# rust-cv/cv

Hardware: NVIDIA H100
Metric: vSLAM frames/s (AKAZE+match+RANSAC, 1080p ~5k kp) at 1/2/4/8 H100 (higher is better)
Workload: dtype f32+f64

## Files before the change

### cv_b200/csrc/arrsac_dev.cuh

```cuda
#pragma once

#define ARS_SORT_CAP 4096u
#define ARS_BOOK_NT 1024
#define ARS_BOOK_SMEM (14u * ARS_SORT_CAP)
#define ARS_QCAP (1u << 20)

struct ArrsacCtl {
    uint32_t n, init_n, Mv, npass;
    uint32_t Hn, cur, blk_lo, blk_hi;
    uint32_t acc_hi, n_new, worst, done;
    uint32_t found, iters, nraw, q_count;
    uint32_t q_count2, stat_lazy;
    uint32_t stat_units0, stat_units2;
    uint32_t stat_repairs, stat_pad;
    uint64_t rng_pos, gen_pos;
    cvb_rng gen;
    cvb_pose winner;
    uint32_t n_inliers, overflow;
    uint32_t stat_chunks, stat_pass;
    uint32_t stat_walk_us, stat_commit_us;
    uint32_t stat_perm_us, stat_turns;
    uint32_t q_blk, stat_qblk;
};

struct ArrsacParams {
    uint32_t K, MM, kind;
    uint32_t H0, ib, bs, max_cand, G;
    uint32_t W0;
    uint32_t NW;
    uint32_t NMAX;
    uint32_t rows;
    uint32_t prefix, cmin;
    float lr_thr, eps0, delta0;
    double thr;
    int row0;
};

__device__ __forceinline__ unsigned long long ars_globaltimer() { unsigned long long t; asm volatile("mov.u64 %0, %%globaltimer;" : "=l"(t)); return t; }
__device__ __forceinline__ uint64_t ars_rotl64(uint64_t x, int k) { return (x << k) | (x >> (64 - k)); }
__device__ uint32_t ars_rng_next_u32(cvb_rng *r) {
    if (r->kind == 0) {
        uint64_t *s = r->s;
        const uint64_t result = ars_rotl64(s[0] + s[3], 23) + s[0];
        const uint64_t t = s[1] << 17;
        s[2] ^= s[0]; s[3] ^= s[1]; s[1] ^= s[2]; s[0] ^= s[3]; s[2] ^= t; s[3] = ars_rotl64(s[3], 45);
        return (uint32_t)(result >> 32);
    }
    unsigned __int128 state = (unsigned __int128)r->s[0] | ((unsigned __int128)r->s[1] << 64);
    const unsigned __int128 incr = (unsigned __int128)r->s[2] | ((unsigned __int128)r->s[3] << 64);
    const unsigned __int128 MUL = ((unsigned __int128)0x2360ED051FC65DA4ull << 64) | 0x4385DF649FCCF645ull;
    state = state * MUL + incr;
    r->s[0] = (uint64_t)state; r->s[1] = (uint64_t)(state >> 64);
    const uint32_t rot = (uint32_t)(state >> 122);
    const uint64_t xsl = (uint64_t)(state >> 64) ^ (uint64_t)state;
    return (uint32_t)((xsl >> rot) | (xsl << ((64 - rot) & 63)));
}

__device__ uint32_t ars_raw_at(ArrsacCtl *ctl, const uint32_t *raw, uint64_t pos) {
    if (pos < ctl->nraw) return raw[pos];
    uint32_t v = 0;
    while (ctl->gen_pos <= pos) { v = ars_rng_next_u32(&ctl->gen); ctl->gen_pos++; }
    return v;
}

#define ARS_WIN 4096u
// ... 150 lines not shown
__global__ void __launch_bounds__(128, MINB) k_ars_estimate8(const ArrsacCtl *ctl, int phase, uint32_t H_init, const double *__restrict__ a,
                                                       const double *__restrict__ b, const uint32_t *__restrict__ samples,
                                                       cvb_pose *poses, uint8_t *nposes) {
    if (ctl->done) return;
    __shared__ double sh[(128 / EIGHT_LANES) * EIGHT_SH];
    const uint32_t H = phase == 0 ? H_init : ctl->n_new;
    const uint32_t g = threadIdx.x / EIGHT_LANES, lane = threadIdx.x % EIGHT_LANES;
    const uint32_t h = blockIdx.x * (128 / EIGHT_LANES) + g;
    if (h >= H) return;
    const unsigned mask = ((1u << EIGHT_LANES) - 1u) << ((threadIdx.x & 31) / EIGHT_LANES * EIGHT_LANES);
    cvb_pose out[4];
    const int n = eight_point_lanes<EIGHT_LANES>(a, b, samples + (size_t)h * 8, out, sh + g * EIGHT_SH, lane, mask);
    if (lane == 0) {
        for (int k = 0; k < n; k++) poses[(size_t)h * 4 + k] = out[k];
        nposes[h] = (uint8_t)n;
    }
}

__device__ __noinline__ bool ars_exact_c2c(const cvb_pose *Pz, const double *pa, const double *pb, double thr) {
    return residual_c2c(*Pz, pa, pb) < thr;
}

template <int RES>
__device__ __forceinline__ bool ars_inlier(const cvb_pose &Pz, const double *__restrict__ a, const double *__restrict__ b, uint32_t i,
                                           double thr) {
    if (RES == 1) return residual_w2c(Pz, a + 3 * (size_t)i, b + 4 * (size_t)i) < thr;
    const double *pa = a + 3 * (size_t)i, *pb = b + 3 * (size_t)i;
    int f = c2c_inlier_filter(Pz.r, Pz.t, pa, pb, thr);
    if (f < 0) f = ars_exact_c2c(&Pz, pa, pb, thr) ? 1 : 0;
    return f != 0;
}

template <int RES>
__device__ __forceinline__ bool ars_inlier_queued(const cvb_pose &Pz, const double *__restrict__ a, const double *__restrict__ b, uint32_t i,
                                                  double thr, uint32_t *qc, uint2 *q, uint32_t src) {
    if (RES == 1) return ars_inlier<RES>(Pz, a, b, i, thr);
    const double *pa = a + 3 * (size_t)i, *pb = b + 3 * (size_t)i;
    const int f = c2c_inlier_filter(Pz.r, Pz.t, pa, pb, thr);
    if (f >= 0) return f != 0;
    const uint32_t slot = atomicAdd(qc, 1u);
    if (slot < ARS_QCAP) { q[slot] = make_uint2(src, i); return false; }
    return ars_exact_c2c(&Pz, pa, pb, thr);
}

__device__ __forceinline__ bool ars_ready(uint32_t word0, uint32_t init_n, uint32_t sample, const ArrsacParams &P) {
    if (sample < P.prefix) return true;
    const uint32_t c = min(32u, init_n);
    return (uint32_t)__popc(c < 32 ? (word0 & ((1u << c) - 1)) : word0) >= P.cmin;
}

template <int RES>
__global__ void __launch_bounds__(256, 2) k_ars_score(ArrsacCtl *ctl, uint2 *__restrict__ queue, ArrsacParams P, int phase, const double *__restrict__ a,
                                                   const double *__restrict__ b, const cvb_pose *__restrict__ poses0,
                                                   const uint8_t *__restrict__ nposes0, uint32_t *__restrict__ masks0,
                                                   const cvb_pose *__restrict__ tposes, uint32_t *__restrict__ tmasks,
                                                   const cvb_pose *__restrict__ newposes, const uint8_t *__restrict__ nposes_new,
                                                   uint32_t *__restrict__ newmask) {
    if (ctl->done) return;
    const unsigned full = 0xffffffffu;
    const uint32_t lane = threadIdx.x & 31;
    const uint32_t warp = (blockIdx.x * blockDim.x + threadIdx.x) >> 5, nwarps = (gridDim.x * blockDim.x) >> 5;
    if (phase == 0 || phase == 2) {
        const uint32_t init_n = ctl->init_n, W = (init_n + 31) >> 5;
        const uint32_t nmod = P.H0 * P.MM, npre = min(P.prefix, P.H0) * P.MM, W1 = W > 0 ? W - 1 : 0;
        const uint32_t units = phase == 0 ? nmod + npre * W1 : (nmod - npre) * W1;
        uint32_t *qc = phase == 0 ? &ctl->q_count : &ctl->q_count2;
        uint2 *q = phase == 0 ? queue : queue + ARS_QCAP;
        for (uint32_t u = warp; u < units; u += nwarps) {
            uint32_t m, w;
            if (phase == 0) { if (u < nmod) { m = u; w = 0; } else { m = (u - nmod) / W1; w = 1 + (u - nmod) % W1; } }
            else { m = npre + u / W1; w = 1 + u % W1; }
            if ((m % P.MM) >= nposes0[m / P.MM]) continue;
            if (phase == 2 && !ars_ready(masks0[(size_t)m * P.W0], init_n, m / P.MM, P)) continue;
            const uint32_t i = w * 32 + lane;
            bool bit = false;
            if (i < init_n) bit = ars_inlier_queued<RES>(poses0[m], a, b, i, P.thr, qc, q, m);
            const unsigned bits = __ballot_sync(full, bit);
            if (lane == 0) { masks0[(size_t)m * P.W0 + w] = bits; atomicAdd(phase == 0 ? &ctl->stat_units0 : &ctl->stat_units2, 1u); }
        }
        return;
    }
    const uint32_t lo = ctl->blk_lo, hi = ctl->blk_hi, Hn = ctl->Hn, cur = ctl->cur;
    const uint32_t wlo = lo >> 5, nwb = hi > lo ? ((hi - 1) >> 5) - wlo + 1 : 0;
    const uint32_t kept_units = Hn * nwb;
    const uint32_t nnew = ctl->n_new * P.MM, nwn = (hi + 31) >> 5;
    const uint32_t units = kept_units + nnew * nwn;
    const cvb_pose *tp = tposes + (size_t)cur * P.rows;
    uint32_t *tm = tmasks + (size_t)cur * P.rows * P.NW;
    for (uint32_t u = warp; u < units; u += nwarps) {
        if (u < kept_units) {
            const uint32_t r = u / nwb, w = wlo + u % nwb;
            const uint32_t i = w * 32 + lane;
            const bool act = i >= lo && i < hi;
            bool bit = false;
            if (act) bit = ars_inlier_queued<RES>(tp[r], a, b, i, P.thr, &ctl->q_blk, queue, r);
            const unsigned bits = __ballot_sync(full, bit), range = __ballot_sync(full, act);
            if (lane == 0) { uint32_t *p = tm + (size_t)r * P.NW + w; *p = (*p & ~range) | bits; }
        } else {
            const uint32_t v = u - kept_units;
            const uint32_t j = v / nwn, w = v % nwn;
            if ((j % P.MM) >= nposes_new[j / P.MM]) continue;
            const uint32_t i = w * 32 + lane;
            bool bit = false;
            if (i < hi) bit = ars_inlier_queued<RES>(newposes[j], a, b, i, P.thr, &ctl->q_blk, queue, P.rows + j);
            const unsigned bits = __ballot_sync(full, bit);
            if (lane == 0) newmask[(size_t)j * P.NW + w] = bits;
        }
    }
}

__global__ void __launch_bounds__(256) k_ars_resolve(const ArrsacCtl *ctl, const uint2 *__restrict__ queue, int stage, ArrsacParams P,
                                                     const double *__restrict__ a, const double *__restrict__ b,
                                                     const cvb_pose *__restrict__ poses0, uint32_t *__restrict__ masks0) {
    if (ctl->done) return;
    const uint32_t cnt = min(stage == 0 ? ctl->q_count : ctl->q_count2, ARS_QCAP);
    queue += stage == 0 ? 0 : ARS_QCAP;
    for (uint32_t e = blockIdx.x * blockDim.x + threadIdx.x; e < cnt; e += gridDim.x * blockDim.x) {
        const uint2 q = queue[e];
        if (residual_c2c(poses0[q.x], a + 3 * (size_t)q.y, b + 3 * (size_t)q.y) < P.thr)
            atomicOr(&masks0[(size_t)q.x * P.W0 + (q.y >> 5)], 1u << (q.y & 31));
    }
}

__global__ void __launch_bounds__(64) k_ars_resolve_block(const ArrsacCtl *ctl, const uint2 *__restrict__ queue, ArrsacParams P,
                                                          const double *__restrict__ a, const double *__restrict__ b,
                                                          const cvb_pose *__restrict__ tposes, uint32_t *__restrict__ tmasks,
                                                          const cvb_pose *__restrict__ newposes, uint32_t *__restrict__ newmask) {
    if (ctl->done) return;
    const uint32_t cnt = min(ctl->q_blk, ARS_QCAP), cur = ctl->cur;
    for (uint32_t e = blockIdx.x * blockDim.x + threadIdx.x; e < cnt; e += gridDim.x * blockDim.x) {
        const uint2 q = queue[e];
        const bool kept = q.x < P.rows;
        const size_t row = kept ? (size_t)cur * P.rows + q.x : (size_t)(q.x - P.rows);
        if (residual_c2c(kept ? tposes[row] : newposes[row], a + 3 * (size_t)q.y, b + 3 * (size_t)q.y) < P.thr)
            atomicOr(&(kept ? tmasks : newmask)[row * P.NW + (q.y >> 5)], 1u << (q.y & 31));
    }
}

__device__ void ars_scan3(uint32_t &a, uint32_t &b, uint32_t &c, uint32_t *sm , uint32_t *tot ) {
    const unsigned full = 0xffffffffu;
    const uint32_t lane = threadIdx.x & 31, wid = threadIdx.x >> 5;
// ... 373 lines not shown
    const uint32_t nsel = ngt + min(neq, need);
    const uint32_t Hn = nsel;
    const uint32_t P2 = ars_pow2(max(Hn, 2u));
    for (uint32_t i = Hn + tid; i < P2; i += NT) keys[i] = ~0ull;
    ars_bitonic(keys, P2);
    for (uint32_t r = tid / 32; r < Hn; r += NT / 32) {
        const uint32_t lane = tid & 31;
        const uint64_t kx = keys[r];
        const uint32_t p = (uint32_t)(kx >> 16) & 0xffffu;
        const uint32_t id = vm[p];
        const double *src = (const double *)(poses0 + id);
        double *dst = (double *)(tposes + r);
        if (lane < 12) dst[lane] = src[lane];
        if (lane == 0) tinl[r] = 0xfffffu - (uint32_t)(kx >> 32);
        for (uint32_t w = lane; w < P.NW; w += 32) tmasks[(size_t)r * P.NW + w] = w < P.W0 ? masks0[(size_t)id * P.W0 + w] : 0u;
    }
    __syncthreads();
    if (tid == 0) {
        const uint32_t n = ctl->n;
        ctl->Hn = Hn; ctl->cur = 0; ctl->stat_pass = npass;
        ctl->acc_hi = init_n; ctl->blk_lo = init_n; ctl->blk_hi = min(init_n + P.bs, n);
        ctl->n_new = 0; ctl->worst = 0;
        if (!(init_n < n && Hn > 1)) {
            ctl->done = 1; ctl->found = Hn >= 1 ? 1 : 0;
            if (Hn >= 1) ctl->winner = tposes[0];
        }
    }
}

__global__ void __launch_bounds__(ARS_BOOK_NT) k_ars_book(ArrsacCtl *ctl, ArrsacParams P, const uint32_t *__restrict__ raw,
                                                           cvb_pose *tposes, uint32_t *tinl, uint32_t *tmasks,
                                                           const cvb_pose *__restrict__ newposes, const uint8_t *__restrict__ nposes_new,
                                                           const uint32_t *__restrict__ newmask, uint32_t *__restrict__ pool,
                                                           uint32_t *__restrict__ samples_new, unsigned long long loop_cond) {
    if (ctl->done) { if (loop_cond && threadIdx.x == 0) cudaGraphSetConditional(loop_cond, 0); return; }
    __shared__ __align__(8) uint32_t sm[96];
    __shared__ uint32_t tot[3];
    extern __shared__ __align__(16) unsigned char ars_dyn[];
    uint64_t *keys = (uint64_t *)ars_dyn;
    uint32_t *e_inl = (uint32_t *)(ars_dyn + 8 * ARS_SORT_CAP);
    uint16_t *e_src = (uint16_t *)(ars_dyn + 12 * ARS_SORT_CAP);
    const uint32_t tid = threadIdx.x, NT = blockDim.x;
    if (tid == 0) { ctl->stat_qblk += ctl->q_blk; ctl->q_blk = 0; }
    const uint32_t cur = ctl->cur, Hk = ctl->Hn, n = ctl->n;
    const uint32_t acc_hi = ctl->acc_hi, lo = ctl->blk_lo, hi = ctl->blk_hi, worst = ctl->worst;
    const uint32_t nnew = ctl->n_new * P.MM;
    const cvb_pose *tp = tposes + (size_t)cur * P.rows;
    const uint32_t *ti = tinl + (size_t)cur * P.rows;
    const uint32_t *tm = tmasks + (size_t)cur * P.rows * P.NW;
    for (uint32_t r = tid; r < Hk; r += NT) { e_inl[r] = ti[r]; e_src[r] = (uint16_t)r; keys[r] = ars_key(ti[r], r, r); }
    uint32_t total = Hk;
    for (uint32_t j0 = 0; j0 < nnew; j0 += NT) {
        const uint32_t j = j0 + tid;
        uint32_t inl = 0;
        bool acc = false;
        if (j < nnew && (j % P.MM) < nposes_new[j / P.MM]) {
            inl = ars_popc_range(newmask + (size_t)j * P.NW, 0, acc_hi);
            acc = inl > worst;
        }
        uint32_t x = acc ? 1 : 0, y = 0, z = 0;
        ars_scan3(x, y, z, sm, tot);
        if (acc) {
            const uint32_t p = total + x - 1;
            if (p < ARS_SORT_CAP) { e_inl[p] = inl; e_src[p] = (uint16_t)(P.rows + j); keys[p] = ars_key(inl, p, p); }
        }
        total += tot[0];
        __syncthreads();
// ... 36 lines not shown
    uint32_t *ni = tinl + (size_t)(cur ^ 1) * P.rows;
    uint32_t *nm = tmasks + (size_t)(cur ^ 1) * P.rows * P.NW;
    const uint32_t nwords = (hi + 31) >> 5;
    for (uint32_t r = tid / 32; r < keep; r += NT / 32) {
        const uint32_t lane = tid & 31;
        const uint32_t e = (uint32_t)keys[r] & 0xffffu;
        const uint32_t src = e_src[e];
        const double *ps = (const double *)(src < P.rows ? tp + src : newposes + (src - P.rows));
        const uint32_t *row = src < P.rows ? tm + (size_t)src * P.NW : newmask + (size_t)(src - P.rows) * P.NW;
        double *pd = (double *)(np_ + r);
        if (lane < 12) pd[lane] = ps[lane];
        if (lane == 0) ni[r] = e_inl[e];
        for (uint32_t w = lane; w < P.NW; w += 32) nm[(size_t)r * P.NW + w] = w < nwords ? row[w] : 0u;
    }
    __syncthreads();
    uint32_t npool = 0;
    for (uint32_t w0 = 0; w0 < nwords; w0 += NT) {
        const uint32_t w = w0 + tid;
        uint32_t x = 0;
        if (w < nwords) {
            x = nm[w];
            if (w * 32 + 32 > hi) x &= ~0u >> (w * 32 + 32 - hi);
        }
        uint32_t c = __popc(x), y = 0, z = 0;
        const uint32_t mine = c;
        ars_scan3(c, y, z, sm, tot);
        uint32_t p = npool + c - mine;
        while (x) { const int b = __ffs(x) - 1; x &= x - 1; pool[p++] = w * 32 + b; }
        npool += tot[0];
        __syncthreads();
    }
    const bool gen = npool >= P.K && P.G > 0;
    if (gen) ars_sample_block(ctl, raw, npool, P.K, P.G, samples_new, pool, (uint32_t *)keys , sm + 64);
    __syncthreads();
    if (tid == 0) {
        ctl->worst = worst_next;
        ctl->n_new = gen ? P.G : 0;
        ctl->cur = cur ^ 1; ctl->Hn = keep;
        ctl->acc_hi = hi; ctl->blk_lo = hi; ctl->blk_hi = min(hi + P.bs, n);
        ctl->iters++;
    }
}

template <int RES>
__global__ void __launch_bounds__(ARS_BOOK_NT) k_ars_final(ArrsacCtl *ctl, ArrsacParams P, const double *__restrict__ a,
                                                            const double *__restrict__ b, cvb_pose *model_out, uint32_t *inliers_out,
                                                            uint32_t cap, uint32_t *n_inliers_out, int32_t *found_out) {
    __shared__ uint32_t sm[96], tot[3];
    const uint32_t tid = threadIdx.x, NT = blockDim.x;
    const uint32_t n = ctl->n;
    const bool found = ctl->found != 0;
    uint32_t cnt = 0;
    if (found) {
        const cvb_pose W = ctl->winner;
        if (tid == 0 && model_out) *model_out = W;
        for (uint32_t i0 = 0; i0 < n; i0 += NT) {
            const uint32_t i = i0 + tid;
            const bool in = i < n && ars_inlier<RES>(W, a, b, i, P.thr);
            uint32_t x = in ? 1 : 0, y = 0, z = 0;
            ars_scan3(x, y, z, sm, tot);
            if (in) { const uint32_t p = cnt + x - 1; if (inliers_out && p < cap) inliers_out[p] = i; }
            cnt += tot[0];
            __syncthreads();
        }
    }
    if (tid == 0) {
        ctl->n_inliers = cnt;
        ctl->overflow = (inliers_out && cnt > cap) ? 1u : 0u;
        if (n_inliers_out) *n_inliers_out = cnt;
        if (found_out) *found_out = found ? 1 : 0;
// ... 3 lines not shown
```

### cv_b200/csrc/geom.cu

```cuda
#include <math.h>
#include <stdio.h>
#include <stdlib.h>
#include <string.h>
#include <algorithm>
#include <vector>
#include "common.cuh"
#include "../../include/cvb200_tri.h"
#include "../../include/cvb200_opt.h"
#include "../../include/cvb200_pinhole.h"
#include "c2c_filter.cuh"
#include "pinhole.cuh"

namespace {

__device__ __forceinline__ void jacobi_cs(double app, double aqq, double apq, double &c, double &s) {
    const double theta = __ddiv_rn(__dsub_rn(aqq, app), __dmul_rn(2.0, apq));
    const double t = __ddiv_rn(theta >= 0.0 ? 1.0 : -1.0, __dadd_rn(fabs(theta), __dsqrt_rn(__dadd_rn(__dmul_rn(theta, theta), 1.0))));
    c = __ddiv_rn(1.0, __dsqrt_rn(__dadd_rn(__dmul_rn(t, t), 1.0)));
    s = __dmul_rn(t, c);
}
__device__ __forceinline__ void jacobi_rot(double &x, double &y, double c, double s) {
    const double a = x, b = y;
    x = __dsub_rn(__dmul_rn(c, a), __dmul_rn(s, b));
    y = __dadd_rn(__dmul_rn(s, a), __dmul_rn(c, b));
// ... 1443 lines not shown
}

__global__ void __launch_bounds__(128) k_essential_decompose(const double *__restrict__ Es, uint32_t m, double eps, int sweeps,
                                                             double *__restrict__ rot_a, double *__restrict__ rot_b, double *__restrict__ t_out,
                                                             uint8_t *__restrict__ ok) {
    const uint32_t j = blockIdx.x * blockDim.x + threadIdx.x;
    if (j >= m) return;
    double E[9], Ra[9], Rb[9], t[3];
    for (int k = 0; k < 9; k++) E[k] = Es[(size_t)j * 9 + k];
    const bool good = essential_rotations(E, eps, sweeps, Ra, Rb, t);
    for (int k = 0; k < 9; k++) { rot_a[(size_t)j * 9 + k] = good ? Ra[k] : none_nan(); rot_b[(size_t)j * 9 + k] = good ? Rb[k] : none_nan(); }
    for (int k = 0; k < 3; k++) t_out[(size_t)j * 3 + k] = good ? t[k] : none_nan();
    ok[j] = good ? 1 : 0;
}

struct DevBuf {
    void *p = nullptr;
    size_t bytes = 0;
    int ensure(cvb_ctx *ctx, size_t need) {
        if (need <= bytes && p) return 0;
        if (p) { cvb_wait(ctx, ctx->stream); cudaFree(p); p = nullptr; bytes = 0; }
        size_t n = std::max<size_t>(need, 256);
        cudaError_t e = cudaMalloc(&p, n);
        if (e != cudaSuccess) return cvb_set_error(ctx, CVB_ENOMEM, "cudaMalloc(%zu): %s", n, cudaGetErrorString(e));
        bytes = n;
        return 0;
    }
};

}

struct ArsWorkspace {
    DevBuf ctl, raw, samples0, poses0, nposes0, masks0, vm, pass_id, pass_inl, tposes, tinl, tmasks, newposes, nposes_new, newmask,
        pool, samples_new, res, queue;
    uint32_t *h_raw = nullptr;
    size_t h_raw_cap = 0;
    unsigned char *h_res = nullptr;
    cudaEvent_t up_done = nullptr;
    std::vector<cvb_rng> snaps;
    cvb_rng rng0;
    uint32_t nraw = 0;
    bool pending = false;
    struct GraphKey {
        ArrsacParams P; int kind, row0; const void *a, *b, *n_dev; uint32_t n_host, nmax, cap, nb; const void *model, *inl, *ninl, *found;
        const void *ws[21];
    };
    struct GraphEntry { GraphKey key; cudaGraphExec_t exec; uint64_t launches; uint32_t body; };
    uint32_t last_body = 0;
    std::vector<GraphEntry> graphs;
    std::vector<GraphKey> seen;
    int use_graph = -1;
    int use_while = -1;
    cudaStream_t body_stream = nullptr;
};
struct GeomWorkspace {
    DevBuf a, b, samples, poses, nposes, out, masks, offsets, ok;
    ArsWorkspace *ars = nullptr;
};
void geom_workspace_free(GeomWorkspace *g) {
    if (!g) return;
    DevBuf *bufs[] = {&g->a, &g->b, &g->samples, &g->poses, &g->nposes, &g->out, &g->masks, &g->offsets, &g->ok};
    for (DevBuf *d : bufs) if (d->p) cudaFree(d->p);
    if (g->ars) {
        ArsWorkspace *w = g->ars;
        DevBuf *ab[] = {&w->ctl, &w->raw, &w->samples0, &w->poses0, &w->nposes0, &w->masks0, &w->vm, &w->pass_id, &w->pass_inl, &w->tposes,
                        &w->tinl, &w->tmasks, &w->newposes, &w->nposes_new, &w->newmask, &w->pool, &w->samples_new, &w->res, &w->queue};
        for (DevBuf *d : ab) if (d->p) cudaFree(d->p);
        if (w->h_raw) cudaFreeHost(w->h_raw);
        if (w->h_res) cudaFreeHost(w->h_res);
        if (w->up_done) cudaEventDestroy(w->up_done);
        if (w->body_stream) cudaStreamDestroy(w->body_stream);
        for (auto &ge : w->graphs) cudaGraphExecDestroy(ge.exec);
        delete w;
    }
    delete g;
}

namespace {
// ... 207 lines not shown
        if ((H[0].mask[i >> 5] >> (i & 31)) & 1u) { if (inliers_out && c < cap) inliers_out[c] = i; c++; }
    if (n_inliers) *n_inliers = c;
    *found = 1;
    (void)nwords;
    if (inliers_out && c > cap) return cvb_set_error(ctx, CVB_ECAP, "inlier capacity %u too small (%u needed)", cap, c);
    return 0;
}


#define ARS_SNAP 4096u
ArsWorkspace *arsws(cvb_ctx *ctx) {
    GeomWorkspace *g = gws(ctx);
    if (!g->ars) g->ars = new ArsWorkspace();
    return g->ars;
}

int arrsac_run_dev(cvb_ctx *ctx, const cvb_arrsac_cfg *cfg, int kind, const double *a_dev, const double *b_dev, const uint32_t *n_dev,
                   uint32_t n_host, uint32_t nmax, const cvb_rng *rng, cvb_pose *model_dev, uint32_t *inl_dev, uint32_t cap,
                   uint32_t *ninl_dev, int32_t *found_dev, int row0) {
    if (cfg->block_size == 0 || cfg->initialization_blocks == 0) return cvb_set_error(ctx, CVB_EINVAL, "block_size / initialization_blocks must be > 0");
    ArrsacParams P;
    memset(&P, 0, sizeof(P));
    P.K = kind_K(kind); P.MM = kind_M(kind); P.kind = (uint32_t)kind;
    P.H0 = cfg->initialization_hypotheses; P.ib = cfg->initialization_blocks; P.bs = cfg->block_size;
    P.max_cand = cfg->max_candidate_hypotheses; P.G = cfg->estimations_per_block;
    P.NMAX = std::max<uint32_t>(nmax, 1);
    P.W0 = cdiv(P.bs * P.ib, 32); P.NW = cdiv(P.NMAX, 32);
    P.rows = P.max_cand + P.G * P.MM;
    P.lr_thr = cfg->likelihood_ratio_threshold; P.eps0 = cfg->initial_epsilon; P.delta0 = cfg->initial_delta;
    P.thr = cfg->inlier_threshold; P.row0 = row0;
    { const char *env = getenv("CVB_ARS_EAGER"); const bool eager = (env && env[0] == '1') || kind_res(kind) == 1;
      P.prefix = eager ? P.H0 : std::min<uint32_t>(P.H0, 64); P.cmin = 2;
      if (const char *cm = getenv("CVB_ARS_CMIN")) P.cmin = (uint32_t)std::max(0, atoi(cm)); }
    if (P.max_cand == 0 || P.rows > ARS_SORT_CAP)
        return cvb_set_error(ctx, CVB_EUNSUPPORTED, "max_candidate_hypotheses + estimations_per_block * %u must be in 1..%u", P.MM, ARS_SORT_CAP);
    if ((uint64_t)P.bs * P.ib + 1 > 2ull * ARS_SORT_CAP) return cvb_set_error(ctx, CVB_EUNSUPPORTED, "block_size * initialization_blocks too large");
    if (P.NMAX >= (1u << 20)) return cvb_set_error(ctx, CVB_EUNSUPPORTED, "more than 2^20 data");
    ArsWorkspace *w = arsws(ctx);
    const uint32_t nb_max = cdiv(P.NMAX, P.bs) + 1;
    const uint32_t nraw = P.H0 * P.K + P.H0 * P.K / 4 + 64 + nb_max * (P.G * P.K + P.G * P.K / 4 + 64);
    const size_t nmodels0 = (size_t)P.H0 * P.MM, nnew = (size_t)std::max<uint32_t>(P.G, 1) * P.MM;
    int rc;
    if ((rc = w->ctl.ensure(ctx, sizeof(ArrsacCtl)))) return rc;
    if ((rc = w->raw.ensure(ctx, sizeof(uint32_t) * (size_t)nraw))) return rc;
    if ((rc = w->samples0.ensure(ctx, sizeof(uint32_t) * (size_t)std::max<uint32_t>(P.H0, 1) * P.K))) return rc;
    if ((rc = w->poses0.ensure(ctx, sizeof(cvb_pose) * std::max<size_t>(nmodels0, 1)))) return rc;
    if ((rc = w->nposes0.ensure(ctx, std::max<uint32_t>(P.H0, 1)))) return rc;
    if ((rc = w->masks0.ensure(ctx, sizeof(uint32_t) * std::max<size_t>(nmodels0, 1) * P.W0))) return rc;
    if ((rc = w->vm.ensure(ctx, sizeof(uint32_t) * std::max<size_t>(nmodels0, ARS_SORT_CAP)))) return rc;
    if ((rc = w->pass_id.ensure(ctx, sizeof(uint32_t) * std::max<size_t>(nmodels0, 1)))) return rc;
    if ((rc = w->pass_inl.ensure(ctx, sizeof(uint32_t) * std::max<size_t>(nmodels0, 1)))) return rc;
    if ((rc = w->tposes.ensure(ctx, sizeof(cvb_pose) * 2 * (size_t)P.rows))) return rc;
    if ((rc = w->tinl.ensure(ctx, sizeof(uint32_t) * 2 * (size_t)P.rows))) return rc;
    if ((rc = w->tmasks.ensure(ctx, sizeof(uint32_t) * 2 * (size_t)P.rows * P.NW))) return rc;
    if ((rc = w->newposes.ensure(ctx, sizeof(cvb_pose) * nnew))) return rc;
    if ((rc = w->nposes_new.ensure(ctx, std::max<uint32_t>(P.G, 1)))) return rc;
    if ((rc = w->newmask.ensure(ctx, sizeof(uint32_t) * nnew * P.NW))) return rc;
    if ((rc = w->pool.ensure(ctx, sizeof(uint32_t) * (size_t)P.NMAX))) return rc;
    if ((rc = w->samples_new.ensure(ctx, sizeof(uint32_t) * (size_t)std::max<uint32_t>(P.G, 1) * P.K))) return rc;
    if ((rc = w->queue.ensure(ctx, sizeof(uint2) * 2 * (size_t)ARS_QCAP))) return rc;
    const size_t hdr = (sizeof(ArrsacCtl) + 15) / 16 * 16, stage_bytes = hdr + sizeof(uint32_t) * (size_t)nraw;
    if (w->h_raw_cap < stage_bytes) {
        if (w->h_raw) { cvb_wait(ctx, ctx->stream); cudaFreeHost(w->h_raw); w->h_raw = nullptr; w->h_raw_cap = 0; }
        if (cudaHostAlloc((void **)&w->h_raw, stage_bytes, cudaHostAllocDefault) != cudaSuccess) return cvb_set_error(ctx, CVB_ENOMEM, "page-locked staging");
        w->h_raw_cap = stage_bytes;
    }
    if (!w->h_res && cudaHostAlloc((void **)&w->h_res, sizeof(ArrsacCtl) + sizeof(cvb_pose) + 64, cudaHostAllocDefault) != cudaSuccess)
        return cvb_set_error(ctx, CVB_ENOMEM, "page-locked staging");
    if (!w->up_done) CVB_CUDA(ctx, cudaEventCreateWithFlags(&w->up_done, cudaEventDisableTiming | cudaEventBlockingSync));
    else CVB_CUDA(ctx, cudaEventSynchronize(w->up_done));
    {
        cvb_rng g = *rng;
        w->rng0 = g;
        w->snaps.clear();
        uint32_t *raw = (uint32_t *)((unsigned char *)w->h_raw + hdr);
        for (uint32_t i = 0; i < nraw; i++) {
            if (i % ARS_SNAP == 0) w->snaps.push_back(g);
            raw[i] = cvb_rng_next_u32(&g);
        }
        ArrsacCtl *h = (ArrsacCtl *)w->h_raw;
        memset(h, 0, sizeof(*h));
        h->nraw = nraw; h->gen = g; h->gen_pos = nraw; h->rng_pos = 0;
        w->nraw = nraw;
    }
    cudaStream_t st = ctx->stream;
    static bool attr_set = false;
    if (!attr_set) {
        cudaFuncSetAttribute(k_ars_book, cudaFuncAttributeMaxDynamicSharedMemorySize, (int)ARS_BOOK_SMEM);
        cudaFuncSetAttribute(k_ars_sprt<0>, cudaFuncAttributeMaxDynamicSharedMemorySize, 64 * 1024);
        cudaFuncSetAttribute(k_ars_sprt<1>, cudaFuncAttributeMaxDynamicSharedMemorySize, 64 * 1024);
// ... 6 lines not shown
    auto enqueue = [&]() -> int {
        CVB_CUDA(ctx, cudaMemcpyAsync(w->ctl.p, w->h_raw, sizeof(ArrsacCtl), cudaMemcpyHostToDevice, st));
        CVB_CUDA(ctx, cudaMemcpyAsync(w->raw.p, (unsigned char *)w->h_raw + hdr, sizeof(uint32_t) * (size_t)nraw, cudaMemcpyHostToDevice, st));
        if (!capturing) CVB_CUDA(ctx, cudaEventRecord(w->up_done, st));
        ArrsacCtl *ctl = (ArrsacCtl *)w->ctl.p;
        const uint32_t *raw = (const uint32_t *)w->raw.p;
        const int res = kind_res(kind);
        {
            CVB_PROF(ctx, "k_ars_begin", 0);
            k_ars_begin<<<1, ARS_BOOK_NT, 0, st>>>(ctl, P, n_dev, n_host, raw, (uint32_t *)w->samples0.p);
            CVB_LAUNCH_CHECK(ctx);
        }
        auto estimate = [&](int phase, uint32_t H, const uint32_t *samples, cvb_pose *poses, uint8_t *nposes) -> int {
            if (H == 0) return 0;
            CVB_PROF(ctx, phase == 0 ? "k_ars_estimate_init" : "k_ars_estimate_block", 0);
            if (kind == 0 && phase == 0) k_ars_estimate8<4, 5><<<cdiv(H, 128 / 4), 128, 0, st>>>(ctl, phase, H, a_dev, b_dev, samples, poses, nposes);
            else if (kind == 0) k_ars_estimate8<16, 5><<<cdiv(H, 128 / 16), 128, 0, st>>>(ctl, phase, H, a_dev, b_dev, samples, poses, nposes);
            else if (kind == 1) k_ars_estimate<1><<<cdiv(H, 128), 128, 0, st>>>(ctl, phase, H, a_dev, b_dev, samples, poses, nposes, row0);
            else k_ars_estimate<2><<<cdiv(H, 128), 128, 0, st>>>(ctl, phase, H, a_dev, b_dev, samples, poses, nposes, row0);
            CVB_LAUNCH_CHECK(ctx);
            return 0;
        };
    const uint32_t sgrid_full = (uint32_t)ctx->num_sms * 4;
        uint32_t sgrid_block = 48;
        if (const char *e = getenv("CVB_ARS_SGRID")) sgrid_block = (uint32_t)std::max(1, atoi(e));
        size_t score_smem = 0;
        if (const char *e = getenv("CVB_ARS_SCORE_SMEM")) score_smem = (size_t)std::max(0, atoi(e));
        auto score = [&](int phase) -> int {
            const uint32_t sgrid = phase == 1 ? sgrid_block : sgrid_full;
            CVB_PROF(ctx, phase == 1 ? "k_ars_score_block" : "k_ars_score_init", 0);
            if (res == 0)
                k_ars_score<0><<<sgrid, 256, score_smem, st>>>(ctl, (uint2 *)w->queue.p, P, phase, a_dev, b_dev, (const cvb_pose *)w->poses0.p, (const uint8_t *)w->nposes0.p,
                                                      (uint32_t *)w->masks0.p, (const cvb_pose *)w->tposes.p, (uint32_t *)w->tmasks.p,
                                                      (const cvb_pose *)w->newposes.p, (const uint8_t *)w->nposes_new.p, (uint32_t *)w->newmask.p);
            else
                k_ars_score<1><<<sgrid, 256, score_smem, st>>>(ctl, (uint2 *)w->queue.p, P, phase, a_dev, b_dev, (const cvb_pose *)w->poses0.p, (const uint8_t *)w->nposes0.p,
                                                      (uint32_t *)w->masks0.p, (const cvb_pose *)w->tposes.p, (uint32_t *)w->tmasks.p,
                                                      (const cvb_pose *)w->newposes.p, (const uint8_t *)w->nposes_new.p, (uint32_t *)w->newmask.p);
            CVB_LAUNCH_CHECK(ctx);
            return 0;
        };
        if ((rc = estimate(0, P.H0, (const uint32_t *)w->samples0.p, (cvb_pose *)w->poses0.p, (uint8_t *)w->nposes0.p))) return rc;
        auto resolve = [&](int stage) -> int {
            CVB_PROF(ctx, "k_ars_resolve", 0);
            k_ars_resolve<<<sgrid_full, 256, 0, st>>>(ctl, (const uint2 *)w->queue.p, stage, P, a_dev, b_dev, (const cvb_pose *)w->poses0.p, (uint32_t *)w->masks0.p);
            CVB_LAUNCH_CHECK(ctx);
            return 0;
        };
        if ((rc = score(0))) return rc;
        if (res == 0 && (rc = resolve(0))) return rc;
        if (P.prefix < P.H0 && P.W0 > 1) {
            if ((rc = score(2))) return rc;
            if (res == 0 && (rc = resolve(1))) return rc;
        }
        {
            CVB_PROF(ctx, "k_ars_sprt", 0);
            if (res == 0)
                k_ars_sprt<0><<<1, ARS_BOOK_NT, 8 * ARS_SORT_CAP, st>>>(ctl, P, a_dev, b_dev, (const cvb_pose *)w->poses0.p, (const uint8_t *)w->nposes0.p, (uint32_t *)w->masks0.p,
                                                        (uint32_t *)w->vm.p, (uint32_t *)w->pass_id.p, (uint32_t *)w->pass_inl.p, (cvb_pose *)w->tposes.p,
                                                        (uint32_t *)w->tinl.p, (uint32_t *)w->tmasks.p);
            else
                k_ars_sprt<1><<<1, ARS_BOOK_NT, 8 * ARS_SORT_CAP, st>>>(ctl, P, a_dev, b_dev, (const cvb_pose *)w->poses0.p, (const uint8_t *)w->nposes0.p, (uint32_t *)w->masks0.p,
                                                        (uint32_t *)w->vm.p, (uint32_t *)w->pass_id.p, (uint32_t *)w->pass_inl.p, (cvb_pose *)w->tposes.p,
                                                        (uint32_t *)w->tinl.p, (uint32_t *)w->tmasks.p);
            CVB_LAUNCH_CHECK(ctx);
        }
        const uint32_t n_bound = n_dev ? P.NMAX : std::min(n_host, P.NMAX);
        const uint32_t init_n = std::min(P.bs * P.ib, n_bound);
        const uint32_t nb = n_bound > init_n ? cdiv(n_bound - init_n, P.bs) : 0;
        auto book = [&](unsigned long long cond) -> int {
            CVB_PROF(ctx, "k_ars_book", 0);
            k_ars_book<<<1, ARS_BOOK_NT, ARS_BOOK_SMEM, st>>>(ctl, P, raw, (cvb_pose *)w->tposes.p, (uint32_t *)w->tinl.p, (uint32_t *)w->tmasks.p,
                                                              (const cvb_pose *)w->newposes.p, (const uint8_t *)w->nposes_new.p,
                                                              (const uint32_t *)w->newmask.p, (uint32_t *)w->pool.p, (uint32_t *)w->samples_new.p, cond);
            CVB_LAUNCH_CHECK(ctx);
            return 0;
        };
        auto score_block = [&](unsigned long long cond) -> int {
            if ((rc = score(1))) return rc;
            if (res == 0) {
                CVB_PROF(ctx, "k_ars_resolve_block", 0);
                k_ars_resolve_block<<<sgrid_full, 64, 0, st>>>(ctl, (const uint2 *)w->queue.p, P, a_dev, b_dev, (const cvb_pose *)w->tposes.p,
                                                               (uint32_t *)w->tmasks.p, (const cvb_pose *)w->newposes.p, (uint32_t *)w->newmask.p);
                CVB_LAUNCH_CHECK(ctx);
            }
            return book(cond);
        };
        if (capturing && while_loop) {
            cudaStreamCaptureStatus cs;
            cudaGraph_t g = nullptr;
            const cudaGraphNode_t *deps = nullptr;
            size_t ndeps = 0;
            CVB_CUDA(ctx, cudaStreamGetCaptureInfo(st, &cs, nullptr, &g, &deps, &ndeps));
            cudaGraphConditionalHandle cond;
            CVB_CUDA(ctx, cudaGraphConditionalHandleCreate(&cond, g, 1, cudaGraphCondAssignDefault));
            cudaGraphNodeParams np = {cudaGraphNodeTypeConditional};
            np.conditional.handle = cond;
            np.conditional.type = cudaGraphCondTypeWhile;
            np.conditional.size = 1;
            cudaGraphNode_t node;
            CVB_CUDA(ctx, cudaGraphAddNode(&node, g, deps, ndeps, &np));
            cudaGraph_t body = np.conditional.phGraph_out[0];
            const cudaStream_t outer = st;
            CVB_CUDA(ctx, cudaStreamBeginCaptureToGraph(w->body_stream, body, nullptr, nullptr, 0, cudaStreamCaptureModeThreadLocal));
            st = w->body_stream;
            const uint64_t b0 = ctx->launches;
            rc = score_block(cond);
// ... 5 lines not shown
            if (rc) return rc;
            CVB_CUDA(ctx, be);
            CVB_CUDA(ctx, cudaStreamUpdateCaptureDependencies(st, &node, 1, cudaStreamSetCaptureDependencies));
        } else
        for (uint32_t it = 0; it <= nb; it++) {
            if ((rc = score_block(0))) return rc;
            if (it < nb && P.G)
                if ((rc = estimate(1, P.G, (const uint32_t *)w->samples_new.p, (cvb_pose *)w->newposes.p, (uint8_t *)w->nposes_new.p))) return rc;
        }
        {
            CVB_PROF(ctx, "k_ars_final", 0);
            if (res == 0) k_ars_final<0><<<1, ARS_BOOK_NT, 0, st>>>(ctl, P, a_dev, b_dev, model_dev, inl_dev, cap, ninl_dev, found_dev);
            else k_ars_final<1><<<1, ARS_BOOK_NT, 0, st>>>(ctl, P, a_dev, b_dev, model_dev, inl_dev, cap, ninl_dev, found_dev);
            CVB_LAUNCH_CHECK(ctx);
        }
        CVB_CUDA(ctx, cudaMemcpyAsync(w->h_res, w->ctl.p, sizeof(ArrsacCtl), cudaMemcpyDeviceToHost, st));
        return 0;
    };
    if (w->use_graph < 0) {
        const char *e1 = getenv("CVB_NO_GRAPH"), *e2 = getenv("CVB_ARS_NO_GRAPH");
        w->use_graph = ((e1 && e1[0] == '1') || (e2 && e2[0] == '1')) ? 0 : 1;
    }
    if (!w->use_graph || ctx->prof) {
        if ((rc = enqueue())) return rc;
        w->pending = true;
        return 0;
    }
    ArsWorkspace::GraphKey key;
    memset(&key, 0, sizeof(key));
    key.P = P; key.kind = kind; key.row0 = row0; key.a = a_dev; key.b = b_dev; key.n_dev = n_dev; key.n_host = n_host; key.nmax = nmax; key.cap = cap;
    key.model = model_dev; key.inl = inl_dev; key.ninl = ninl_dev; key.found = found_dev;
    {
        const DevBuf *bufs[] = {&w->ctl, &w->raw, &w->samples0, &w->poses0, &w->nposes0, &w->masks0, &w->vm, &w->pass_id, &w->pass_inl, &w->tposes,
                                &w->tinl, &w->tmasks, &w->newposes, &w->nposes_new, &w->newmask, &w->pool, &w->samples_new, &w->queue};
        int i = 0;
        for (const DevBuf *d : bufs) key.ws[i++] = d->p;
        key.ws[i++] = w->h_raw; key.ws[i++] = w->h_res; key.ws[i++] = (const void *)(uintptr_t)nraw;
    }
    auto same = [](const ArsWorkspace::GraphKey &x, const ArsWorkspace::GraphKey &y) { return memcmp(&x, &y, sizeof(x)) == 0; };
    for (auto &ge : w->graphs)
        if (same(ge.key, key)) {
            CVB_CUDA(ctx, cudaGraphLaunch(ge.exec, st));
            CVB_CUDA(ctx, cudaEventRecord(w->up_done, st));
            ctx->launches += ge.launches;
            w->last_body = ge.body;
            w->pending = true;
            return 0;
        }
    bool seen = false;
    for (auto &k : w->seen) seen = seen || same(k, key);
    if (!seen) {
        if (w->seen.size() >= 64) w->seen.erase(w->seen.begin());
        w->seen.push_back(key);
        if ((rc = enqueue())) return rc;
        w->pending = true;
        return 0;
    }
    const uint64_t l0 = ctx->launches;
    if (w->use_while < 0) {
        const char *e = getenv("CVB_ARS_WHILE");
        w->use_while = (e && e[0] == '0') ? 0 : 1;
    }
    if (w->use_while && !w->body_stream && cudaStreamCreateWithFlags(&w->body_stream, cudaStreamNonBlocking) != cudaSuccess) {
        cudaGetLastError();
        w->use_while = 0;
    }
    cudaGraphExec_t exec = nullptr;
// ... 9 lines not shown
        capturing = false;
        if (!rc && ce == cudaSuccess && graph) ce = cudaGraphInstantiate(&exec, graph, 0);
        if (graph) cudaGraphDestroy(graph);
        if (exec || !while_loop) break;
        cudaGetLastError();
        w->use_while = 0;
        exec = nullptr;
    }
    if (rc) return rc;
    if (ce != cudaSuccess || !exec) {
        cudaGetLastError();
        w->use_graph = 0;
        ctx->launches = l0;
        if ((rc = enqueue())) return rc;
        w->pending = true;
        return 0;
    }
    if (w->graphs.size() >= 16) { cudaGraphExecDestroy(w->graphs.front().exec); w->graphs.erase(w->graphs.begin()); }
    w->graphs.push_back({key, exec, ctx->launches - l0, while_loop ? body_launches : 0u});
    w->last_body = while_loop ? body_launches : 0u;
    CVB_CUDA(ctx, cudaGraphLaunch(exec, st));
    CVB_CUDA(ctx, cudaEventRecord(w->up_done, st));
    w->pending = true;
    return 0;
}

int arrsac_commit_rng(cvb_ctx *ctx, cvb_rng *rng, ArrsacCtl *stats_out = nullptr) {
    ArsWorkspace *w = arsws(ctx);
    if (!w->pending) return cvb_set_error(ctx, CVB_EINVAL, "no device ARRSAC run to commit");
    const ArrsacCtl *h = (const ArrsacCtl *)w->h_res;
    if (stats_out) *stats_out = *h;
    if (getenv("CVB_ARS_DEBUG"))
        fprintf(stderr, "[arrsac] n %u models %u pass %u chunks %u turns %u repairs %u lazy %u | sprt us: order %u walk %u commit %u | block iterations %u"
                " | undecided predicates queued: initial %u block %u\n", h->n, h->Mv, h->npass, h->stat_chunks, h->stat_turns, h->stat_repairs,
                h->stat_lazy, h->stat_perm_us, h->stat_walk_us, h->stat_commit_us, h->iters, h->q_count + h->q_count2, h->stat_qblk);
    ctx->launches += (uint64_t)w->last_body * h->iters;
    w->last_body = 0;
    w->pending = false;
    if (!rng) return 0;
    const uint64_t used = h->rng_pos;
    if (used >= w->nraw) {
        if (h->gen_pos != std::max<uint64_t>(used, w->nraw)) return cvb_set_error(ctx, CVB_ECUDA, "generator position mismatch");
        *rng = h->gen;
        return 0;
    }
    cvb_rng g = w->snaps[used / ARS_SNAP];
    for (uint64_t i = used / ARS_SNAP * ARS_SNAP; i < used; i++) cvb_rng_next_u32(&g);
    *rng = g;
    return 0;
}

int arrsac_host(cvb_ctx *ctx, const cvb_arrsac_cfg *cfg, int kind, const double *a, const double *b, uint32_t n, cvb_rng *rng,
                cvb_pose *model_out, uint32_t *inliers_out, uint32_t cap, uint32_t *n_inliers, int32_t *found, int row0 = 5) {
    *found = 0;
    if (n_inliers) *n_inliers = 0;
    if (n < kind_K(kind) || cfg->initialization_hypotheses == 0) return 0;
    CVB_CUDA(ctx, cudaSetDevice(ctx->device));
    int rc = upload_data(ctx, kind, a, b, n);
    if (rc) return rc;
    GeomWorkspace *g = gws(ctx);
    ArsWorkspace *w = arsws(ctx);
    const size_t res_bytes = sizeof(cvb_pose) + 16 + sizeof(uint32_t) * (size_t)n;
    if ((rc = w->res.ensure(ctx, res_bytes))) return rc;
    unsigned char *rd = (unsigned char *)w->res.p;
    cvb_pose *model_dev = (cvb_pose *)rd;
    uint32_t *ninl_dev = (uint32_t *)(rd + sizeof(cvb_pose));
    int32_t *found_dev = (int32_t *)(rd + sizeof(cvb_pose) + 4);
    uint32_t *inl_dev = (uint32_t *)(rd + sizeof(cvb_pose) + 16);
// ... 654 lines not shown
```

Baseline: 1538.

## Early-reject new ARRSAC hypotheses that cannot beat the current worst kept model

Adds a per-new-hypothesis outlier counter that the block scoring kernel updates atomically. Once a hypothesis has more confirmed outliers over the prefix than the bar (lo minus worst inlier count), its remaining word units are skipped and zero-filled. The book kernel also stops generating new hypotheses when the worst kept model already covers the whole block, and it resets the counters each iteration. Work-unit ordering for new hypotheses changes to word-major so early prefix words are scored first, at the cost of extra atomics, a global load per unit, and added debug statistics.

```diff
diff --git a/cv_b200/csrc/arrsac_dev.cuh b/cv_b200/csrc/arrsac_dev.cuh
--- a/cv_b200/csrc/arrsac_dev.cuh
+++ b/cv_b200/csrc/arrsac_dev.cuh
@@ -21,6 +21,10 @@
     uint32_t stat_walk_us, stat_commit_us;
     uint32_t stat_perm_us, stat_turns;
     uint32_t q_blk, stat_qblk;
+    uint32_t stat_units_kept, stat_units_new;
+    uint32_t stat_skip;
+    uint32_t stat_blk_w0, stat_blk_lt32;
+    uint32_t stat_blk_bar0;
 };
 
 struct ArrsacParams {
@@ -31,6 +35,7 @@
     uint32_t NMAX;
     uint32_t rows;
     uint32_t prefix, cmin;
+    uint32_t early;
     float lr_thr, eps0, delta0;
     double thr;
     int row0;
@@ -247,15 +252,15 @@
 }
 
 template <int RES>
-__device__ __forceinline__ bool ars_inlier_queued(const cvb_pose &Pz, const double *__restrict__ a, const double *__restrict__ b, uint32_t i,
-                                                  double thr, uint32_t *qc, uint2 *q, uint32_t src) {
-    if (RES == 1) return ars_inlier<RES>(Pz, a, b, i, thr);
+__device__ __forceinline__ int ars_inlier_queued(const cvb_pose &Pz, const double *__restrict__ a, const double *__restrict__ b, uint32_t i,
+                                                 double thr, uint32_t *qc, uint2 *q, uint32_t src) {
+    if (RES == 1) return ars_inlier<RES>(Pz, a, b, i, thr) ? 1 : 0;
     const double *pa = a + 3 * (size_t)i, *pb = b + 3 * (size_t)i;
     const int f = c2c_inlier_filter(Pz.r, Pz.t, pa, pb, thr);
-    if (f >= 0) return f != 0;
+    if (f >= 0) return f != 0 ? 1 : 0;
     const uint32_t slot = atomicAdd(qc, 1u);
-    if (slot < ARS_QCAP) { q[slot] = make_uint2(src, i); return false; }
-    return ars_exact_c2c(&Pz, pa, pb, thr);
+    if (slot < ARS_QCAP) { q[slot] = make_uint2(src, i); return -1; }
+    return ars_exact_c2c(&Pz, pa, pb, thr) ? 1 : 0;
 }
 
 __device__ __forceinline__ bool ars_ready(uint32_t word0, uint32_t init_n, uint32_t sample, const ArrsacParams &P) {
@@ -270,7 +275,7 @@
                                                    const uint8_t *__restrict__ nposes0, uint32_t *__restrict__ masks0,
                                                    const cvb_pose *__restrict__ tposes, uint32_t *__restrict__ tmasks,
                                                    const cvb_pose *__restrict__ newposes, const uint8_t *__restrict__ nposes_new,
-                                                   uint32_t *__restrict__ newmask) {
+                                                   uint32_t *__restrict__ newmask, uint32_t *nout) {
     if (ctl->done) return;
     const unsigned full = 0xffffffffu;
     const uint32_t lane = threadIdx.x & 31;
@@ -289,39 +294,60 @@
             if (phase == 2 && !ars_ready(masks0[(size_t)m * P.W0], init_n, m / P.MM, P)) continue;
             const uint32_t i = w * 32 + lane;
             bool bit = false;
-            if (i < init_n) bit = ars_inlier_queued<RES>(poses0[m], a, b, i, P.thr, qc, q, m);
+            if (i < init_n) bit = ars_inlier_queued<RES>(poses0[m], a, b, i, P.thr, qc, q, m) > 0;
             const unsigned bits = __ballot_sync(full, bit);
             if (lane == 0) { masks0[(size_t)m * P.W0 + w] = bits; atomicAdd(phase == 0 ? &ctl->stat_units0 : &ctl->stat_units2, 1u); }
         }
         return;
     }
     const uint32_t lo = ctl->blk_lo, hi = ctl->blk_hi, Hn = ctl->Hn, cur = ctl->cur;
+    const uint32_t worst = ctl->worst;
     const uint32_t wlo = lo >> 5, nwb = hi > lo ? ((hi - 1) >> 5) - wlo + 1 : 0;
     const uint32_t kept_units = Hn * nwb;
     const uint32_t nnew = ctl->n_new * P.MM, nwn = (hi + 31) >> 5;
     const uint32_t units = kept_units + nnew * nwn;
     const cvb_pose *tp = tposes + (size_t)cur * P.rows;
     uint32_t *tm = tmasks + (size_t)cur * P.rows * P.NW;
+    const uint32_t bar = lo > worst ? lo - worst : 0;
+    if (blockIdx.x == 0 && threadIdx.x == 0) {
+        uint32_t valid = 0;
+        for (uint32_t s = 0; s < ctl->n_new; s++) valid += min((uint32_t)nposes_new[s], P.MM);
+        ctl->stat_units_kept += kept_units; ctl->stat_units_new += valid * nwn;
+        if (nnew) { ctl->stat_blk_w0 += worst == 0; ctl->stat_blk_lt32 += bar < 32; }
+    }
+    uint32_t skipped = 0;
     for (uint32_t u = warp; u < units; u += nwarps) {
-        if (u < kept_units) {
-            const uint32_t r = u / nwb, w = wlo + u % nwb;
-            const uint32_t i = w * 32 + lane;
-            const bool act = i >= lo && i < hi;
-            bool bit = false;
-            if (act) bit = ars_inlier_queued<RES>(tp[r], a, b, i, P.thr, &ctl->q_blk, queue, r);
-            const unsigned bits = __ballot_sync(full, bit), range = __ballot_sync(full, act);
-            if (lane == 0) { uint32_t *p = tm + (size_t)r * P.NW + w; *p = (*p & ~range) | bits; }
+        const bool kept = u < kept_units;
+        uint32_t src, w;
+        if (kept) { src = u / nwb; w = wlo + u % nwb; }
+        else {
+            const uint32_t v = u - kept_units, j = v % nnew;
+            if ((j % P.MM) >= nposes_new[j / P.MM]) continue;
+            src = P.rows + j; w = v / nnew;
+            if (P.early && __ldcg(nout + j) >= bar) {
+                if (lane == 0) newmask[(size_t)j * P.NW + w] = 0u;
+                skipped++;
+                continue;
+            }
+        }
+        const uint32_t i = w * 32 + lane;
+        const bool act = i < hi && (!kept || i >= lo);
+        int f = -1;
+        if (act) f = ars_inlier_queued<RES>(kept ? tp[src] : newposes[src - P.rows], a, b, i, P.thr, &ctl->q_blk, queue, src);
+        const unsigned bits = __ballot_sync(full, f > 0);
+        if (kept) {
+            const unsigned range = __ballot_sync(full, act);
+            if (lane == 0) { uint32_t *p = tm + (size_t)src * P.NW + w; *p = (*p & ~range) | bits; }
         } else {
-            const uint32_t v = u - kept_units;
-            const uint32_t j = v / nwn, w = v % nwn;
-            if ((j % P.MM) >= nposes_new[j / P.MM]) continue;
-            const uint32_t i = w * 32 + lane;
-            bool bit = false;
-            if (i < hi) bit = ars_inlier_queued<RES>(newposes[j], a, b, i, P.thr, &ctl->q_blk, queue, P.rows + j);
-            const unsigned bits = __ballot_sync(full, bit);
-            if (lane == 0) newmask[(size_t)j * P.NW + w] = bits;
-        }
-    }
+            const uint32_t j = src - P.rows;
+            const unsigned out = __ballot_sync(full, f == 0 && i < lo);
+            if (lane == 0) {
+                newmask[(size_t)j * P.NW + w] = bits;
+                if (P.early && out) atomicAdd(nout + j, (uint32_t)__popc(out));
+            }
+        }
+    }
+    if (lane == 0 && skipped) atomicAdd(&ctl->stat_skip, skipped);
 }
 
 __global__ void __launch_bounds__(256) k_ars_resolve(const ArrsacCtl *ctl, const uint2 *__restrict__ queue, int stage, ArrsacParams P,
@@ -761,7 +787,8 @@
                                                            cvb_pose *tposes, uint32_t *tinl, uint32_t *tmasks,
                                                            const cvb_pose *__restrict__ newposes, const uint8_t *__restrict__ nposes_new,
                                                            const uint32_t *__restrict__ newmask, uint32_t *__restrict__ pool,
-                                                           uint32_t *__restrict__ samples_new, unsigned long long loop_cond) {
+                                                           uint32_t *__restrict__ samples_new, uint32_t *__restrict__ nout,
+                                                           unsigned long long loop_cond) {
     if (ctl->done) { if (loop_cond && threadIdx.x == 0) cudaGraphSetConditional(loop_cond, 0); return; }
     __shared__ __align__(8) uint32_t sm[96];
     __shared__ uint32_t tot[3];
@@ -864,10 +891,13 @@
     }
     const bool gen = npool >= P.K && P.G > 0;
     if (gen) ars_sample_block(ctl, raw, npool, P.K, P.G, samples_new, pool, (uint32_t *)keys , sm + 64);
+    for (uint32_t j = tid; j < P.G * P.MM; j += NT) nout[j] = 0;
     __syncthreads();
     if (tid == 0) {
+        const bool bar0 = worst_next >= hi;
         ctl->worst = worst_next;
-        ctl->n_new = gen ? P.G : 0;
+        ctl->n_new = gen && !bar0 ? P.G : 0;
+        ctl->stat_blk_bar0 += gen && bar0;
         ctl->cur = cur ^ 1; ctl->Hn = keep;
         ctl->acc_hi = hi; ctl->blk_lo = hi; ctl->blk_hi = min(hi + P.bs, n);
         ctl->iters++;
diff --git a/cv_b200/csrc/geom.cu b/cv_b200/csrc/geom.cu
--- a/cv_b200/csrc/geom.cu
+++ b/cv_b200/csrc/geom.cu
@@ -1499,7 +1499,7 @@
 
 struct ArsWorkspace {
     DevBuf ctl, raw, samples0, poses0, nposes0, masks0, vm, pass_id, pass_inl, tposes, tinl, tmasks, newposes, nposes_new, newmask,
-        pool, samples_new, res, queue;
+        nout, pool, samples_new, res, queue;
     uint32_t *h_raw = nullptr;
     size_t h_raw_cap = 0;
     unsigned char *h_res = nullptr;
@@ -1510,7 +1510,7 @@
     bool pending = false;
     struct GraphKey {
         ArrsacParams P; int kind, row0; const void *a, *b, *n_dev; uint32_t n_host, nmax, cap, nb; const void *model, *inl, *ninl, *found;
-        const void *ws[21];
+        const void *ws[22];
     };
     struct GraphEntry { GraphKey key; cudaGraphExec_t exec; uint64_t launches; uint32_t body; };
     uint32_t last_body = 0;
@@ -1784,6 +1784,7 @@
     { const char *env = getenv("CVB_ARS_EAGER"); const bool eager = (env && env[0] == '1') || kind_res(kind) == 1;
       P.prefix = eager ? P.H0 : std::min<uint32_t>(P.H0, 64); P.cmin = 2;
       if (const char *cm = getenv("CVB_ARS_CMIN")) P.cmin = (uint32_t)std::max(0, atoi(cm)); }
+    { const char *e = getenv("CVB_ARS_EARLY_REJECT"); P.early = (e && e[0] == '0') ? 0u : 1u; }
     if (P.max_cand == 0 || P.rows > ARS_SORT_CAP)
         return cvb_set_error(ctx, CVB_EUNSUPPORTED, "max_candidate_hypotheses + estimations_per_block * %u must be in 1..%u", P.MM, ARS_SORT_CAP);
     if ((uint64_t)P.bs * P.ib + 1 > 2ull * ARS_SORT_CAP) return cvb_set_error(ctx, CVB_EUNSUPPORTED, "block_size * initialization_blocks too large");
@@ -1808,6 +1809,7 @@
     if ((rc = w->newposes.ensure(ctx, sizeof(cvb_pose) * nnew))) return rc;
     if ((rc = w->nposes_new.ensure(ctx, std::max<uint32_t>(P.G, 1)))) return rc;
     if ((rc = w->newmask.ensure(ctx, sizeof(uint32_t) * nnew * P.NW))) return rc;
+    if ((rc = w->nout.ensure(ctx, sizeof(uint32_t) * nnew))) return rc;
     if ((rc = w->pool.ensure(ctx, sizeof(uint32_t) * (size_t)P.NMAX))) return rc;
     if ((rc = w->samples_new.ensure(ctx, sizeof(uint32_t) * (size_t)std::max<uint32_t>(P.G, 1) * P.K))) return rc;
     if ((rc = w->queue.ensure(ctx, sizeof(uint2) * 2 * (size_t)ARS_QCAP))) return rc;
@@ -1880,11 +1882,13 @@
             if (res == 0)
                 k_ars_score<0><<<sgrid, 256, score_smem, st>>>(ctl, (uint2 *)w->queue.p, P, phase, a_dev, b_dev, (const cvb_pose *)w->poses0.p, (const uint8_t *)w->nposes0.p,
                                                       (uint32_t *)w->masks0.p, (const cvb_pose *)w->tposes.p, (uint32_t *)w->tmasks.p,
-                                                      (const cvb_pose *)w->newposes.p, (const uint8_t *)w->nposes_new.p, (uint32_t *)w->newmask.p);
+                                                      (const cvb_pose *)w->newposes.p, (const uint8_t *)w->nposes_new.p, (uint32_t *)w->newmask.p,
+                                                      (uint32_t *)w->nout.p);
             else
                 k_ars_score<1><<<sgrid, 256, score_smem, st>>>(ctl, (uint2 *)w->queue.p, P, phase, a_dev, b_dev, (const cvb_pose *)w->poses0.p, (const uint8_t *)w->nposes0.p,
                                                       (uint32_t *)w->masks0.p, (const cvb_pose *)w->tposes.p, (uint32_t *)w->tmasks.p,
-                                                      (const cvb_pose *)w->newposes.p, (const uint8_t *)w->nposes_new.p, (uint32_t *)w->newmask.p);
+                                                      (const cvb_pose *)w->newposes.p, (const uint8_t *)w->nposes_new.p, (uint32_t *)w->newmask.p,
+                                                      (uint32_t *)w->nout.p);
             CVB_LAUNCH_CHECK(ctx);
             return 0;
         };
@@ -1920,7 +1924,8 @@
             CVB_PROF(ctx, "k_ars_book", 0);
             k_ars_book<<<1, ARS_BOOK_NT, ARS_BOOK_SMEM, st>>>(ctl, P, raw, (cvb_pose *)w->tposes.p, (uint32_t *)w->tinl.p, (uint32_t *)w->tmasks.p,
                                                               (const cvb_pose *)w->newposes.p, (const uint8_t *)w->nposes_new.p,
-                                                              (const uint32_t *)w->newmask.p, (uint32_t *)w->pool.p, (uint32_t *)w->samples_new.p, cond);
+                                                              (const uint32_t *)w->newmask.p, (uint32_t *)w->pool.p, (uint32_t *)w->samples_new.p,
+                                                              (uint32_t *)w->nout.p, cond);
             CVB_LAUNCH_CHECK(ctx);
             return 0;
         };
@@ -1992,7 +1997,7 @@
     key.model = model_dev; key.inl = inl_dev; key.ninl = ninl_dev; key.found = found_dev;
     {
         const DevBuf *bufs[] = {&w->ctl, &w->raw, &w->samples0, &w->poses0, &w->nposes0, &w->masks0, &w->vm, &w->pass_id, &w->pass_inl, &w->tposes,
-                                &w->tinl, &w->tmasks, &w->newposes, &w->nposes_new, &w->newmask, &w->pool, &w->samples_new, &w->queue};
+                                &w->tinl, &w->tmasks, &w->newposes, &w->nposes_new, &w->newmask, &w->nout, &w->pool, &w->samples_new, &w->queue};
         int i = 0;
         for (const DevBuf *d : bufs) key.ws[i++] = d->p;
         key.ws[i++] = w->h_raw; key.ws[i++] = w->h_res; key.ws[i++] = (const void *)(uintptr_t)nraw;
@@ -2068,8 +2073,10 @@
     if (stats_out) *stats_out = *h;
     if (getenv("CVB_ARS_DEBUG"))
         fprintf(stderr, "[arrsac] n %u models %u pass %u chunks %u turns %u repairs %u lazy %u | sprt us: order %u walk %u commit %u | block iterations %u"
-                " | undecided predicates queued: initial %u block %u\n", h->n, h->Mv, h->npass, h->stat_chunks, h->stat_turns, h->stat_repairs,
-                h->stat_lazy, h->stat_perm_us, h->stat_walk_us, h->stat_commit_us, h->iters, h->q_count + h->q_count2, h->stat_qblk);
+                " | undecided predicates queued: initial %u block %u | block units: kept %u new %u skipped %u | blocks worst0 %u bar<32 %u not estimated %u\n",
+                h->n, h->Mv, h->npass, h->stat_chunks, h->stat_turns, h->stat_repairs, h->stat_lazy, h->stat_perm_us, h->stat_walk_us,
+                h->stat_commit_us, h->iters, h->q_count + h->q_count2, h->stat_qblk, h->stat_units_kept, h->stat_units_new, h->stat_skip,
+                h->stat_blk_w0, h->stat_blk_lt32, h->stat_blk_bar0);
     ctx->launches += (uint64_t)w->last_body * h->iters;
     w->last_body = 0;
     w->pending = false;
```

Measured after the change: 1603 (median of 6 runs). 1.04x the previous value.
